# indygreg/python-zstandard

Measured on NVIDIA H100. Metric: uncompressed GB/s (compress+decompress), higher is better.
Workload: dtype u8

## Files before the change

### python_zstandard_b200/csrc/zb_common.cuh

```cuda
#pragma once
#include <cstdint>
#include <cstring>
#include <cuda_runtime.h>

typedef uint8_t  u8;
typedef uint16_t u16;
typedef uint32_t u32;
typedef uint64_t u64;

enum : u32 {
    ZB_OK = 0,
    ZB_E_GENERIC = 1,
    ZB_E_PREFIX_UNKNOWN = 10,
    ZB_E_FRAMEPARAM_UNSUPPORTED = 14,
    ZB_E_WINDOW_TOO_LARGE = 16,
    ZB_E_CORRUPTION = 20,
    ZB_E_CHECKSUM_WRONG = 22,
    ZB_E_LITERALS_HEADER_WRONG = 24,
    ZB_E_DICT_CORRUPTED = 30,
    ZB_E_DICT_WRONG = 32,
    ZB_E_TABLELOG_TOO_LARGE = 44,
    ZB_E_MAXSYMBOL_TOO_SMALL = 48,
    ZB_E_MEMORY = 64,
    ZB_E_DSTSIZE_TOO_SMALL = 70,
// ... 139 lines not shown
};

typedef uint4 ZbSeq;

typedef u32 ZbFseCell;
#define ZB_CELL(next, nb, add, sym) ((u32)(next) | ((u32)(nb) << 10) | ((u32)(add) << 14) | ((u32)(sym) << 19))
#define ZB_CELL_NEXT(c) ((c) & 1023u)
#define ZB_CELL_NB(c)   (((c) >> 10) & 15u)
#define ZB_CELL_ADD(c)  (((c) >> 14) & 31u)
#define ZB_CELL_SYM(c)  ((c) >> 19)
#define ZB_CELL16(sym, x) ((u16)((sym) | ((x) << 6)))

struct ZbDictDev {
    const u8* content; u32 content_size; u32 dict_id;
    const u16* huf; u32 huf_log; u32 has_entropy;
    const ZbFseCell* ll; const ZbFseCell* of; const ZbFseCell* ml;
    u32 ll_log, of_log, ml_log;
    u32 rep[3];
};

struct ZbDictDigest {
    u16 huf[4096]; ZbFseCell ll[512]; ZbFseCell ml[512]; ZbFseCell of[256];
    u32 huf_log, ll_log, of_log, ml_log; u32 rep[3]; u32 dict_id; u32 content_off; u32 status; u32 has_entropy; u32 pad;
    short c_norm_ll[36], c_norm_of[32], c_norm_ml[54]; u32 c_max_ll, c_max_of, c_max_ml;
    u8 c_huf_nb[256]; u32 c_huf_max;
};

__device__ __forceinline__ u32 zb_rd16(const u8* p) { return (u32)p[0] | ((u32)p[1] << 8); }
__device__ __forceinline__ u32 zb_rd24(const u8* p) { return zb_rd16(p) | ((u32)p[2] << 16); }
__device__ __forceinline__ u32 zb_rd32(const u8* p) { return zb_rd16(p) | (zb_rd16(p + 2) << 16); }
__device__ __forceinline__ u64 zb_rd64(const u8* p) { return (u64)zb_rd32(p) | ((u64)zb_rd32(p + 4) << 32); }
__device__ __forceinline__ int zb_hibit(u32 v) { return 31 - __clz(v); }

__device__ __forceinline__ void zb_cp16(u8* sdst, const u8* gsrc)
{
#ifdef __CUDA_ARCH__
    asm volatile("cp.async.cg.shared.global [%0], [%1], 16;" :: "r"((u32)__cvta_generic_to_shared(sdst)), "l"(gsrc) : "memory");
#else
    memcpy(sdst, gsrc, 16);
#endif
}
__device__ __forceinline__ void zb_cp_commit()
{
#ifdef __CUDA_ARCH__
    asm volatile("cp.async.commit_group;" ::: "memory");
#endif
}
template <int N> __device__ __forceinline__ void zb_cp_wait()
{
#ifdef __CUDA_ARCH__
    asm volatile("cp.async.wait_group %0;" :: "n"(N) : "memory");
#endif
}

#ifdef __CUDA_ARCH__
#define ZB_RING_ARG(name) u8* name
#else
#define ZB_RING_ARG(name) u8* name = nullptr
#endif
template <int D>
struct ZbBitR {
    static_assert(D >= 2 && (D & (D - 1)) == 0, "ring depth: a power of two");
    const u8* c; u8* ring; int widx; u32 hi, lo; int avail; u32 nx0, nx1; int skew_bits; int lo_c; u32 n_;
#ifndef __CUDA_ARCH__
    alignas(16) u8 own[16 * D];
#endif

    __device__ __forceinline__ u32 word(int j) const { return *(const u32*)(ring + ((u32)j & (4u * D - 1)) * 4u); }
    __device__ __forceinline__ void fetch(int k) { zb_cp16(ring + ((u32)k & (D - 1)) * 16u, c + 16 * k); }
    __device__ __forceinline__ ~ZbBitR() { zb_cp_wait<0>(); }

    __device__ __forceinline__ bool start(const u8* s, u32 n, u8* ring_) {
        if (n == 0) return false;
#ifdef __CUDA_ARCH__
        ring = ring_;
#else
        ring = ring_ ? ring_ : own;
#endif
        c = (const u8*)((uintptr_t)s & ~(uintptr_t)15);
        int const skew = (int)(s - c);
        skew_bits = skew * 8; n_ = n;
        int const top = (skew + (int)n - 1) >> 4;
        #pragma unroll
        for (int q = 0; q < D; q++) if (top - q >= 0) fetch(top - q);
        zb_cp_commit();
        lo_c = top - D + 1 > 0 ? top - D + 1 : 0;
        return true;
    }
    __device__ __forceinline__ bool finish() {
        zb_cp_wait<0>();
        int const e = skew_bits / 8 + (int)n_ - 1;
        u32 const last = ring[(u32)e & (16u * D - 1)];
        if (last == 0) return false;
        int const P = e * 8 + zb_hibit(last);
        nx0 = nx1 = 0; lo = 0;
        if (P == 0) { hi = 0; avail = 0; widx = -1; return true; }
        int const wi = (P - 1) >> 5, k = P - wi * 32;
        hi = word(wi) << (32 - k); avail = k; widx = wi - 1;
        if (widx >= 0) nx0 = word(widx);
        if (widx >= 1) nx1 = word(widx - 1);
        refill();
        return true;
    }
    __device__ __forceinline__ bool init(const u8* s, u32 n, u8* ring_) { return start(s, n, ring_) && finish(); }
    __device__ __forceinline__ void refill() {
        zb_cp_wait<4 * D - 8>();
        bool const r = (avail <= 32) & (widx >= 0);
        u32 const a = (u32)avail;
        u32 const add_hi = __funnelshift_rc(nx0, 0u, a);
        u32 const new_lo = __funnelshift_lc(0u, nx0, 32u - a);
        hi |= r ? add_hi : 0u;
        lo = r ? new_lo : lo;
        avail += r ? 32 : 0;
        widx -= r ? 1 : 0;
        nx0 = r ? nx1 : nx0;
        if (r && widx >= 1) nx1 = word(widx - 1);
        int const t = ((widx - 1) >> 2) + 1 - D;
        if (t >= 0 && t < lo_c) { fetch(t); lo_c = t; }
        zb_cp_commit();
    }
    __device__ __forceinline__ u32 peek(u32 nb) const { return __funnelshift_rc(hi, 0u, 32u - nb); }
    __device__ __forceinline__ void skip(u32 nb) {
        hi = __funnelshift_lc(lo, hi, nb); lo = __funnelshift_lc(0u, lo, nb); avail -= (int)nb;
    }
    __device__ __forceinline__ u32 read(u32 nb) { u32 const v = peek(nb); skip(nb); return v; }
    __device__ __forceinline__ int left() const { return avail + 32 * (widx + 1) - skew_bits; }
};
```

### python_zstandard_b200/csrc/zb_entropy.cuh

```cuda
#pragma once

#define ZB_ENT_WS_BYTES   256
#define ZB_ENT_WS_STRIDE  (ZB_ENT_WS_BYTES + 16)
#define ZB_ENT_SKEW(b)    ((((b) + 15u) & ~15u) | 16u)
#define ZB_ENT_DEF_LL     512
#define ZB_ENT_DEF_OF     (ZB_ENT_DEF_LL + 2 * 64)
#define ZB_ENT_DEF_ML     (ZB_ENT_DEF_OF + 2 * 32)
#define ZB_ENT_HEAD_BYTES (ZB_ENT_DEF_ML + 2 * 64)
#define ZB_ENT_POOL_BYTES(W) ((((227 * 1024 - ZB_ENT_HEAD_BYTES) / (W))) & ~15)
#define ZB_ENT_SMEM(W)    ((W) * ZB_ENT_POOL_BYTES(W) + ZB_ENT_HEAD_BYTES)

enum : u32 { ZB_SRC_NONE = 0, ZB_SRC_PREDEF = 1, ZB_SRC_RLE = 2, ZB_SRC_NCOUNT = 3, ZB_SRC_DICT = 4 };
struct ZbTabSrc { u32 kind; u32 sym; const u8* p; u32 n; };

enum : u32 { ZB_BD_FIRST = 1, ZB_BD_FSE_VALID = 2, ZB_BD_SKIP = 4 };
struct ZbBlkDesc {
    u64 hdr_off;
    u64 seq_off, lit_off;
    u32 span;
    u32 frame;
    u32 flags;
    u32 block_max;
    ZbTabSrc dHuf, dLL, dOF, dML;
};
// ... 62 lines not shown
            u32 const sy = wt[u], x = (u32)(u16)norm[sy]; norm[sy] = (short)(x + 1);
            u32 const nb = log - (u32)zb_hibit(x);
            wt[u] = (u16)(sy | (nb << 4) | (((x << nb) - size) << 8));
        }
        clear_nibbles();
        ZbBitR<4> b;
        if (!b.init(s + 1 + used, hdr - used, ring)) return 0;
        u32 s1 = b.read(log), s2 = b.read(log); b.refill();
        if (b.left() < 0) return 0;
        nsym = 0;
        for (;;) {
            if (nsym + 2 > 255) return 0;
            { u32 c = wt[s1], w = c & 15; if (w > 12) return 0; put(nsym, w); rank.count(w); total += (1u << w) >> 1; nsym++;
              s1 = (c >> 8) + b.read((c >> 4) & 15); b.refill(); }
            if (b.left() < 0) { u32 w = wt[s2] & 15; if (w > 12) return 0; put(nsym, w); rank.count(w); total += (1u << w) >> 1; nsym++; break; }
            if (nsym + 2 > 255) return 0;
            { u32 c = wt[s2], w = c & 15; if (w > 12) return 0; put(nsym, w); rank.count(w); total += (1u << w) >> 1; nsym++;
              s2 = (c >> 8) + b.read((c >> 4) & 15); b.refill(); }
            if (b.left() < 0) { u32 w = wt[s1] & 15; if (w > 12) return 0; put(nsym, w); rank.count(w); total += (1u << w) >> 1; nsym++; break; }
        }
    }
    if (total == 0) return 0;
    u32 const log = (u32)zb_hibit(total) + 1;
    if (log > 12) return 0;
    u32 const rest = (1u << log) - total, hb = (u32)zb_hibit(rest);
    if ((1u << hb) != rest) return 0;
    put(nsym, hb + 1); rank.count(hb + 1); nsym++;
    if (rank[1] < 2 || (rank[1] & 1)) return 0;
    out_log = log; out_nsym = nsym;
    return hdr + 1;
}

#define ZB_HUF_COARSE 8u
struct ZbHufTab { const u16* cells; u32 log, shift, T, base; };
__device__ __forceinline__ void zb_huf_shape(u32 log, ZbRank const& rank, u32& shift, u32& T, u32& base, u32& bytes)
{
    shift = log > ZB_HUF_COARSE ? log - ZB_HUF_COARSE : 0u;
    T = 0;
    #pragma unroll
    for (u32 wt = 1; wt <= 12 - ZB_HUF_COARSE; wt++) T += wt <= shift ? rank[wt] << (wt - 1) : 0u;
    base = (T + 3u) & ~3u;
    bytes = 2u * (base + (1u << (log - shift)));
}
__device__ __forceinline__ ZbHufTab zb_huf_full(const u16* cells, u32 log) { ZbHufTab t; t.cells = cells; t.log = log; t.shift = 0; t.T = 0; t.base = 0; return t; }
#define ZB_HCELL(t, v) ((t).cells[(v) < (t).T ? (v) : (t).base + ((v) >> (t).shift)])

__device__ static void zb_huf_fill(u16* cells, const u8* ws, u32 log, u32 nsym, ZbRank const& rank, u32 shift, u32 base)
{
    ZbPacked<6, 16> next; next.clear();
    {
        u32 p = 0;
        #pragma unroll
        for (u32 wt = 1; wt <= 12; wt++) { next.add(wt - 1, p); p += wt <= log ? (rank[wt] << (wt - 1)) : 0; }
    }
    for (u32 i = 0; i < nsym; i++) {
        u32 const wt = (ws[i >> 1] >> ((i & 1) * 4)) & 15; if (!wt) continue;
        u32 len = 1u << (wt - 1), p = next.get(wt - 1); next.add(wt - 1, len);
        if (wt > shift) { len >>= shift; p = base + (p >> shift); }
        u32 const cell = i | ((log + 1 - wt) << 8);
        if (len >= 4) { u64 const v = cell * 0x0001000100010001ull; u64* q = (u64*)(cells + p); for (u32 k = 0; k < len / 4; k++) q[k] = v; }
        else if (len == 2) *(u32*)(cells + p) = cell * 0x00010001u;
        else cells[p] = (u16)cell;
    }
}

#ifdef ZB_SIMT_EMULATION
__device__ __forceinline__ ZbRank zb_rank_pack(const u32* rank) { ZbRank r; r.clear(); for (u32 wt = 1; wt <= 12; wt++) r.add(wt - 1, rank[wt]); return r; }
__device__ static u32 zb_huf_weights(u8* ws, const u8* s, u32 n, u32& out_log, u32& out_nsym, u32* rank, ZB_RING_ARG(ring))
{
    ZbRank r; u32 const used = zb_huf_weights(ws, s, n, out_log, out_nsym, r, ring);
    rank[0] = used ? out_nsym : 0;
    for (u32 w = 1; w <= 12; w++) { rank[w] = used ? r[w] : 0; rank[0] -= rank[w]; }
    return used;
}
__device__ __forceinline__ void zb_huf_shape(u32 log, const u32* rank, u32& shift, u32& T, u32& base, u32& bytes)
{
    zb_huf_shape(log, zb_rank_pack(rank), shift, T, base, bytes);
}
__device__ static void zb_huf_fill(u16* cells, const u8* ws, u32 log, u32 nsym, const u32* rank, u32 shift, u32 base)
{
    zb_huf_fill(cells, ws, log, nsym, zb_rank_pack(rank), shift, base);
}
#endif

__device__ static bool zb_huf_stream2(u8* out, u32 n_out, const u8* s, u32 n, ZbHufTab const t, u8* ring)
{
    ZbBitR<4> b;
    if (!b.init(s, n, ring)) return false;
    u32 const log = t.log;
    u32 i = 0;
    while (i < n_out && ((uintptr_t)(out + i) & 3)) { u32 v = b.peek(log); u32 c = ZB_HCELL(t, v); out[i++] = (u8)c; b.skip(c >> 8); b.refill(); }
    for (; i + 4 <= n_out; i += 4) {
        u32 v0 = b.peek(log); u32 c0 = ZB_HCELL(t, v0); b.skip(c0 >> 8);
        u32 v1 = b.peek(log); u32 c1 = ZB_HCELL(t, v1); b.skip(c1 >> 8); b.refill();
        u32 v2 = b.peek(log); u32 c2 = ZB_HCELL(t, v2); b.skip(c2 >> 8);
        u32 v3 = b.peek(log); u32 c3 = ZB_HCELL(t, v3); b.skip(c3 >> 8); b.refill();
        *(u32*)(out + i) = (c0 & 255) | ((c1 & 255) << 8) | ((c2 & 255) << 16) | (c3 << 24);
    }
    for (; i < n_out; i++) { u32 v = b.peek(log); u32 c = ZB_HCELL(t, v); out[i] = (u8)c; b.skip(c >> 8); b.refill(); }
    return b.left() == 0;
}

struct ZbHufLane { ZbBitR<4> b; u8* out; u32 left; };

__device__ __forceinline__ void zb_huf_one(ZbHufLane& h, ZbHufTab const& t)
{
    u32 const v = h.b.peek(t.log); u32 const c = ZB_HCELL(t, v); *h.out++ = (u8)c; h.b.skip(c >> 8); h.b.refill(); h.left--;
}
#define ZB_HUF4(h) do { \
        u32 const v0_ = h.b.peek(t.log); u32 const c0_ = ZB_HCELL(t, v0_); h.b.skip(c0_ >> 8); \
        u32 const v1_ = h.b.peek(t.log); u32 const c1_ = ZB_HCELL(t, v1_); h.b.skip(c1_ >> 8); h.b.refill(); \
        u32 const v2_ = h.b.peek(t.log); u32 const c2_ = ZB_HCELL(t, v2_); h.b.skip(c2_ >> 8); \
        u32 const v3_ = h.b.peek(t.log); u32 const c3_ = ZB_HCELL(t, v3_); h.b.skip(c3_ >> 8); h.b.refill(); \
        *(u32*)h.out = (c0_ & 255) | ((c1_ & 255) << 8) | ((c2_ & 255) << 16) | (c3_ << 24); h.out += 4; h.left -= 4; } while (0)

__device__ static bool zb_huf_block(u8* dstl, u32 regen, const u8* p, u32 left, bool single, ZbHufTab const t, ZB_RING_ARG(ring))
{
    if (single) return zb_huf_stream2(dstl, regen, p, left, t, ring);
    if (left < 10) return false;
    u32 const l1 = zb_rd16(p), l2 = zb_rd16(p + 2), l3 = zb_rd16(p + 4), seg = (regen + 3) / 4;
    if (6 + l1 + l2 + l3 > left || seg * 3 > regen) return false;
    u32 const l4 = left - 6 - l1 - l2 - l3;
    ZbHufLane h0, h1, h2, h3;
    u8* const r1 = ring ? ring + 64 : nullptr; u8* const r2 = ring ? ring + 128 : nullptr; u8* const r3 = ring ? ring + 192 : nullptr;
    if (!h0.b.start(p + 6, l1, ring) || !h1.b.start(p + 6 + l1, l2, r1) || !h2.b.start(p + 6 + l1 + l2, l3, r2) || !h3.b.start(p + 6 + l1 + l2 + l3, l4, r3)) return false;
    if (!h0.b.finish() || !h1.b.finish() || !h2.b.finish() || !h3.b.finish()) return false;
    h0.out = dstl; h1.out = dstl + seg; h2.out = dstl + 2 * seg; h3.out = dstl + 3 * seg;
    h0.left = h1.left = h2.left = seg; h3.left = regen - 3 * seg;
    while (h0.left && ((uintptr_t)h0.out & 3)) zb_huf_one(h0, t);
    while (h1.left && ((uintptr_t)h1.out & 3)) zb_huf_one(h1, t);
    while (h2.left && ((uintptr_t)h2.out & 3)) zb_huf_one(h2, t);
    while (h3.left && ((uintptr_t)h3.out & 3)) zb_huf_one(h3, t);
    while (h0.left >= 4 && h1.left >= 4 && h2.left >= 4 && h3.left >= 4) { ZB_HUF4(h0); ZB_HUF4(h1); ZB_HUF4(h2); ZB_HUF4(h3); }
    while (h0.left >= 4) ZB_HUF4(h0);
    while (h1.left >= 4) ZB_HUF4(h1);
    while (h2.left >= 4) ZB_HUF4(h2);
    while (h3.left >= 4) ZB_HUF4(h3);
    while (h0.left) zb_huf_one(h0, t);
    while (h1.left) zb_huf_one(h1, t);
    while (h2.left) zb_huf_one(h2, t);
    while (h3.left) zb_huf_one(h3, t);
    return h0.b.left() == 0 && h1.b.left() == 0 && h2.b.left() == 0 && h3.b.left() == 0;
}

__device__ static int zb_seq_desc(ZbTabSrc& d, u32 mode, u32 max_sym_kind, u32 max_log, const u8* ip, u32 avail,
                                  bool repeat_ok, short* norm, u32& log, u32& max_sym, u32& need)
{
    int used = 0;
    if (mode == 0) { d.kind = ZB_SRC_PREDEF; }
    else if (mode == 1) { if (avail == 0 || ip[0] > max_sym_kind) return -1; d.kind = ZB_SRC_RLE; d.sym = ip[0]; used = 1; }
    else if (mode == 2) { d.kind = ZB_SRC_NCOUNT; d.p = ip; d.n = avail; }
    else if (!repeat_ok || d.kind == ZB_SRC_NONE) return -1;
    need = 0; log = 0; max_sym = max_sym_kind;
    if (d.kind == ZB_SRC_NCOUNT) {
        u32 const u = zb_read_ncount(norm, max_sym, log, d.p, d.n);
        if (u == 0 || log > max_log) return -1;
        if (mode == 2) { used = (int)u; d.n = u; }
        need = 2u << log;
    } else if (d.kind == ZB_SRC_RLE) need = 2;
    return used;
}

template <class F> __device__ __forceinline__ void zb_cta_for(u32 n, F f)
{
#ifdef __CUDA_ARCH__
    for (u32 i = threadIdx.x; i < n; i += blockDim.x) f(i);
#else
    if (threadIdx.x == 0) for (u32 i = 0; i < n; i++) f(i);
#endif
}

__device__ __forceinline__ void zb_cta_cells16(u8* dst, const ZbFseCell* src, u32 log)
{
    zb_cta_for(1u << log, [&](u32 i) { u32 const c = src[i]; ((u16*)dst)[i] = ZB_CELL16(ZB_CELL_SYM(c), (ZB_CELL_NEXT(c) + (1u << log)) >> ZB_CELL_NB(c)); });
}

template <int W>
__device__ __forceinline__ u32 zb_ent_head(u8* smem, ZbDictDev const& dict)
{
    u32* const lutLL = (u32*)smem; u32* const lutML = lutLL + 36;
    zb_cta_for(36, [&](u32 i) { lutLL[i] = c_LL_base[i] | ((u32)c_LL_bits[i] << 24); });
    zb_cta_for(53, [&](u32 i) { lutML[i] = c_ML_base[i] | ((u32)c_ML_bits[i] << 24); });
    zb_cta_cells16(smem + ZB_ENT_DEF_LL, g_defLL, 6);
    zb_cta_cells16(smem + ZB_ENT_DEF_OF, g_defOF, 5);
    zb_cta_cells16(smem + ZB_ENT_DEF_ML, g_defML, 6);
    u32 head = ZB_ENT_HEAD_BYTES;
    if (dict.has_entropy) {
        zb_cta_cells16(smem + head, dict.ll, dict.ll_log); head += 2u << dict.ll_log;
        zb_cta_cells16(smem + head, dict.of, dict.of_log); head += 2u << dict.of_log;
        zb_cta_cells16(smem + head, dict.ml, dict.ml_log); head += 2u << dict.ml_log;
    }
    __syncthreads();
    return ((ZB_ENT_SMEM(W) - head) / W) & ~15u;
}

#ifdef ZB_PHASE_TIMERS
__device__ unsigned long long g_zb_ent_phase[8];
#define ZB_EMARK(k) do { if (lane == 0) { long long const t_ = clock64(); atomicAdd(&g_zb_ent_phase[k], (unsigned long long)(t_ - t_ph)); t_ph = t_; } } while (0)
#elif defined(ZB_DEBUG_BLOCKS)
#define ZB_EMARK(k) do { if (err && !(t_ph & 1)) { printf("[emark %d] lane %u err %u\n", k, lane, err); t_ph |= 1; } } while (0)
#else
#define ZB_EMARK(k) do { (void)t_ph; } while (0)
#endif

template <bool SYMREP>
__device__ __forceinline__ u32 zb_seq_block(const u8* smem, u8* q, u8* ws, ZbDictDev const& dict,
                                            ZbTabSrc const& dLL, ZbTabSrc const& dOF, ZbTabSrc const& dML,
                                            u32 msLL, u32 msOF, u32 msML, u32 logLL, u32 logOF, u32 logML,
                                            const u8* ip, const u8* bend, u32 nseq, ZbSeq* sq, u32 n_lit, u64 room, u64 hist,
                                            u32& rep0, u32& rep1, u32& rep2, u32& lit_used, u32& produced, long long& t_ph)
{
    const u32* const lutLL = (const u32*)smem; const u32* const lutML = lutLL + 36;
    short* const normLL = (short*)ws; short* const normOF = normLL + 36; short* const normML = normOF + 32;
    u32 const dct_ll = ZB_ENT_HEAD_BYTES, dct_of = dct_ll + (2u << dict.ll_log), dct_ml = dct_of + (2u << dict.of_log);
    ZbTab tLL, tOF, tML;
    auto setup = [&](const ZbTabSrc& d, short* norm, u32 ms, u32 lg, int kind, u32 dct, u32 dlog, u32 def, u32 deflog, ZbTab& t) {
        if (d.kind == ZB_SRC_NCOUNT) { zb_build_fse((u16*)q, norm, ms, lg, kind); t.off = (u32)(q - smem); t.log = lg; q += 2u << lg; }
        else if (d.kind == ZB_SRC_RLE) { *(u16*)q = ZB_CELL16(d.sym, 1u); t.off = (u32)(q - smem); t.log = 0; q += 2; }
        else if (d.kind == ZB_SRC_DICT) { t.off = dct; t.log = dlog; }
        else { t.off = def; t.log = deflog; }
    };
    setup(dLL, normLL, msLL, logLL, K_LL, dct_ll, dict.ll_log, ZB_ENT_DEF_LL, 6, tLL);
    setup(dOF, normOF, msOF, logOF, K_OF, dct_of, dict.of_log, ZB_ENT_DEF_OF, 5, tOF);
// ... 40 lines not shown
        if (slow) b.refill();
        {
            u32 const both = b.read(ab);
            ml += both >> llb; ll += both & ((1u << llb) - 1);
        }
        if (slow) b.refill();
        {
            u32 const v = b.read(sb);
            sLL = (xl << nl) - (1u << tLL.log) + (v >> (nm + no));
            sML = (xm << nm) - (1u << tML.log) + ((v >> no) & ((1u << nm) - 1));
            sOF = (xo << no) - (1u << tOF.log) + (v & ((1u << no) - 1));
        }
        sq[i] = make_uint4(lit_used, produced, ml, off);
        if ((u64)produced + ll + ml > room) { err = ZB_E_DSTSIZE_TOO_SMALL; break; }
        if (ll > n_lit - lit_used) { err = ZB_E_CORRUPTION; break; }
        lit_used += ll; produced += ll;
        if ((u64)off > hist + produced) { err = ZB_E_CORRUPTION; break; }
        produced += ml;
    }
    if (!err && b.left() != 0) err = ZB_E_CORRUPTION;
    return err;
}

template <int ZB_ENT_WARPS>
__global__ void __launch_bounds__(ZB_ENT_WARPS * 32)
zb_entropy_decode(const u8* __restrict__ src, const ZbSegment* __restrict__ segs, u32 n_frames,
                  const ZbFramePlace* __restrict__ place, const u64* __restrict__ dst_sizes,
                  ZbBlock* __restrict__ blocks, ZbSeq* __restrict__ seqs, u8* __restrict__ lits,
                  u32* __restrict__ work_counter, ZbDictDev dict, u32* status, u64* __restrict__ out_sizes,
                  u32* __restrict__ ck_expect, u32 take)
{
    ZB_DYN_SMEM(zb_smem);
    u32 const lane = threadIdx.x & 31, warp = threadIdx.x >> 5;
    u32 const pool_bytes = zb_ent_head<ZB_ENT_WARPS>(zb_smem, dict);
    u8* const pool = zb_smem + ZB_ENT_SMEM(ZB_ENT_WARPS) - (ZB_ENT_WARPS - warp) * pool_bytes;
    u8* const ws = pool + lane * ZB_ENT_WS_STRIDE;
    u8* const tabs = pool + 32 * ZB_ENT_WS_STRIDE;
    u32 const TAB_BYTES = pool_bytes - 32 * ZB_ENT_WS_STRIDE;

    for (;;) {
        u32 base = 0;
        if (lane == 0) base = atomicAdd(work_counter, take);
        base = __shfl_sync(0xFFFFFFFFu, base, 0);
        if (base >= n_frames) return;
        u32 const f = base + lane;
        bool done = lane >= take || !(f < n_frames) || status[f] != ZB_OK;

        const u8* s = src; u64 n = 0; ZbHdr h; ZbFramePlace pl; u32 err = ZB_OK;
        u64 cap = 0, out_pos = 0, blk_i = 0, seq_i = 0, lit_i = 0, pos = 0; u32 block_max = 0;
        u32 rep0 = 1, rep1 = 4, rep2 = 8;
        ZbTabSrc dHuf = {ZB_SRC_NONE, 0, nullptr, 0}, dLL = dHuf, dOF = dHuf, dML = dHuf;
        bool fse_valid = false;
        if (!done) {
            s = src + segs[f].offset; n = segs[f].length;
            zb_skip_skippable(s, n);
            zb_parse_header(s, n, h);
            pl = place[f]; cap = pl.dst_cap; blk_i = pl.blk_off; seq_i = pl.seq_off; lit_i = pl.lit_off; pos = h.hdr_size;
            block_max = h.window < ZB_BLOCK_MAX ? (u32)h.window : ZB_BLOCK_MAX;
            if (dict.has_entropy) {
                dHuf.kind = dLL.kind = dOF.kind = dML.kind = ZB_SRC_DICT; fse_valid = true;
                rep0 = dict.rep[0]; rep1 = dict.rep[1]; rep2 = dict.rep[2];
            }
            if (h.dict_id && dict.dict_id && h.dict_id != dict.dict_id) { err = ZB_E_DICT_WRONG; done = true; }
        }
        u64 const hist_extra = dict.content_size;

        long long t_ph = clock64() & ~1ll;
// ... 28 lines not shown
                        B.n_lit = L.regen; comp = true;
                    }
                } while (0);
                if (err) { done = true; comp = false; }
            }
            ZB_EMARK(1);
            bool wantH = false; u32 hlog = 0, hns = 0; ZbRank rank; const u8* hp = nullptr; u32 hleft = 0;
            if (comp) {
                do {
                    if (L.type == 0) {
                        if (L.hdr + L.regen > bsize) { err = ZB_E_CORRUPTION; break; }
                        B.lit_kind = ZB_LIT_RAW; B.src_pos = (u64)(bs + L.hdr - src); ip = bs + L.hdr + L.regen;
                    } else if (L.type == 1) {
                        if (L.hdr + 1 > bsize) { err = ZB_E_CORRUPTION; break; }
                        B.lit_kind = ZB_LIT_RLE; B.lit_byte = bs[L.hdr]; ip = bs + L.hdr + 1;
                    } else {
                        if (L.type == 3 && dHuf.kind == ZB_SRC_NONE) { err = ZB_E_DICT_CORRUPTED; break; }
                        if (!L.single && L.regen < 6) { err = ZB_E_LITERALS_HEADER_WRONG; break; }
                        if (L.csize + L.hdr > bsize || L.regen == 0) { err = ZB_E_CORRUPTION; break; }
                        hp = bs + L.hdr; hleft = L.csize;
                        if (L.type == 2) { dHuf.kind = ZB_SRC_NCOUNT; dHuf.p = hp; dHuf.n = hleft; }
                        if (dHuf.kind == ZB_SRC_NCOUNT) {
                            u32 const used = zb_huf_weights(ws, dHuf.p, dHuf.n, hlog, hns, rank, tabs + lane * 80);
                            if (used == 0 || (L.type == 2 && used >= hleft)) { err = ZB_E_CORRUPTION; break; }
                            if (L.type == 2) { hp += used; hleft -= used; dHuf.n = used; }
                            wantH = true;
                        }
                        B.lit_kind = ZB_LIT_SCRATCH; B.src_pos = lit_i; ip = bs + L.hdr + L.csize;
                    }
                } while (0);
                if (err) { done = true; comp = false; wantH = false; }
            }
            if (comp && B.lit_kind == ZB_LIT_SCRATCH && dHuf.kind == ZB_SRC_DICT) {
                if (!zb_huf_block(lits + lit_i, L.regen, hp, hleft, L.single, zb_huf_full(dict.huf, dict.huf_log), ws)) { err = ZB_E_CORRUPTION; done = true; comp = false; }
            }
            ZB_EMARK(2);
            {
                bool pending = wantH;
                u32 hshift = 0, hT = 0, hbase = 0, hbytes = 0;
                if (wantH) zb_huf_shape(hlog, rank, hshift, hT, hbase, hbytes);
                while (__any_sync(0xFFFFFFFFu, pending)) {
                    u32 const need = pending ? hbytes : 0;
                    u32 const incl = zb_warp_incl_scan((need + 15) & ~15u, lane);
                    if (pending && incl <= TAB_BYTES) {
                        u16* cells = (u16*)(tabs + incl - ((need + 15) & ~15u));
                        zb_huf_fill(cells, ws, hlog, hns, rank, hshift, hbase);
                        ZB_EMARK(6);
                        ZbHufTab t; t.cells = cells; t.log = hlog; t.shift = hshift; t.T = hT; t.base = hbase;
                        if (!zb_huf_block(lits + lit_i, L.regen, hp, hleft, L.single, t, ws)) { err = ZB_E_CORRUPTION; done = true; comp = false; }
                        pending = false;
                    }
                    __syncwarp();
                }
            }
            ZB_EMARK(3);
            if (comp && B.lit_kind == ZB_LIT_SCRATCH) lit_i += (L.regen + 15) & ~15u;
            u32 nseq = 0, logLL = 0, logOF = 0, logML = 0, msLL = 0, msOF = 0, msML = 0, needS = 0;
            short* const normLL = (short*)ws; short* const normOF = normLL + 36; short* const normML = normOF + 32;
            if (comp) {
                do {
                    if (ip >= bend) { err = ZB_E_SRCSIZE_WRONG; break; }
                    nseq = *ip++;
                    if (nseq > 0x7F) {
                        if (nseq == 0xFF) { if (ip + 2 > bend) { err = ZB_E_SRCSIZE_WRONG; break; } nseq = zb_rd16(ip) + 0x7F00; ip += 2; }
                        else { if (ip >= bend) { err = ZB_E_SRCSIZE_WRONG; break; } nseq = ((nseq - 0x80) << 8) + *ip++; }
                    }
                    B.n_seq = nseq;
                    if (nseq == 0) { if (ip != bend) err = ZB_E_CORRUPTION; break; }
                    if (ip + 1 > bend) { err = ZB_E_SRCSIZE_WRONG; break; }
                    u32 const modes = *ip++;
                    if (modes & 3) { err = ZB_E_CORRUPTION; break; }
                    u32 nd; int r;
                    r = zb_seq_desc(dLL, modes >> 6, 35, 9, ip, (u32)(bend - ip), fse_valid, normLL, logLL, msLL, nd);
                    if (r < 0) { err = ZB_E_CORRUPTION; break; } ip += r; needS += nd;
                    r = zb_seq_desc(dOF, (modes >> 4) & 3, 31, 8, ip, (u32)(bend - ip), fse_valid, normOF, logOF, msOF, nd);
                    if (r < 0) { err = ZB_E_CORRUPTION; break; } ip += r; needS += nd;
                    r = zb_seq_desc(dML, (modes >> 2) & 3, 52, 9, ip, (u32)(bend - ip), fse_valid, normML, logML, msML, nd);
                    if (r < 0) { err = ZB_E_CORRUPTION; break; } ip += r; needS += nd;
                    fse_valid = true;
                } while (0);
                if (err) { done = true; comp = false; nseq = 0; }
// ... 26 lines not shown
                    if (!err && B.regen > block_max) err = ZB_E_CORRUPTION;
                    pos += bsize;
                }
                if (!err) {
                    blocks[blk_i++] = B;
                    out_pos += B.regen;
                    if (last) {
                        if (h.content_size != ZB_CONTENT_UNKNOWN && out_pos != h.content_size) err = ZB_E_CORRUPTION;
                        else if (h.checksum && pos + 4 > n) err = ZB_E_CHECKSUM_WRONG;
                        else {
                            if (h.checksum) ck_expect[f] = zb_rd32(s + pos);
                            if (dst_sizes && out_pos != cap) err = ZB_E_SIZE_MISMATCH;
                        }
                        done = true;
                    }
                }
                if (err) done = true;
            }
        }
        if (lane < take && f < n_frames && status[f] == ZB_OK) {
            if (err) { status[f] = err; out_sizes[f] = err == ZB_E_SIZE_MISMATCH ? out_pos : 0; } else out_sizes[f] = out_pos;
        } else if (lane < take && f < n_frames) out_sizes[f] = 0;
    }
}

template <int ZB_ENT_WARPS>
__global__ void __launch_bounds__(ZB_ENT_WARPS * 32)
zb_entropy_blocks(const u8* __restrict__ src, const ZbBlkDesc* __restrict__ bdesc, u32 n_blocks,
                  ZbBlock* __restrict__ blocks, ZbSeq* __restrict__ seqs, u8* __restrict__ lits,
                  u32* __restrict__ work_counter, ZbDictDev dict, u32* status, ZbBlkExit* __restrict__ bexit, u32 take)
{
    ZB_DYN_SMEM(zb_smem);
    u32 const lane = threadIdx.x & 31, warp = threadIdx.x >> 5;
    u32 const pool_bytes = zb_ent_head<ZB_ENT_WARPS>(zb_smem, dict);
    u8* const pool = zb_smem + ZB_ENT_SMEM(ZB_ENT_WARPS) - (ZB_ENT_WARPS - warp) * pool_bytes;
    u8* const ws = pool + lane * ZB_ENT_WS_BYTES;
    u8* const tabs = pool + 32 * ZB_ENT_WS_BYTES;
    u32 const TAB_BYTES = pool_bytes - 32 * ZB_ENT_WS_BYTES;

    for (;;) {
        u32 base = 0;
        if (lane == 0) base = atomicAdd(work_counter, take);
        base = __shfl_sync(0xFFFFFFFFu, base, 0);
        if (base >= n_blocks) return;
        u32 const bi = base + lane;
        ZbBlkDesc D; D.frame = 0; D.flags = 0;
        if (lane < take && bi < n_blocks) D = bdesc[bi];
        bool done = lane >= take || !(bi < n_blocks) || (D.flags & ZB_BD_SKIP) || status[D.frame] != ZB_OK;

        const u8* s = src; u64 n = 0; u32 err = ZB_OK;
        u64 const cap = ~0ull >> 1; u64 out_pos = 0, blk_i = bi, seq_i = 0, lit_i = 0, pos = 0; u32 block_max = 0;
        u32 rep0 = 1, rep1 = 4, rep2 = 8;
        ZbTabSrc dHuf = {ZB_SRC_NONE, 0, nullptr, 0}, dLL = dHuf, dOF = dHuf, dML = dHuf;
        bool fse_valid = false;
        if (!done) {
            s = src + D.hdr_off; n = D.span; seq_i = D.seq_off; lit_i = D.lit_off; block_max = D.block_max;
            dHuf = D.dHuf; dLL = D.dLL; dOF = D.dOF; dML = D.dML; fse_valid = (D.flags & ZB_BD_FSE_VALID) != 0;
            if (D.flags & ZB_BD_FIRST) { if (dict.has_entropy) { rep0 = dict.rep[0]; rep1 = dict.rep[1]; rep2 = dict.rep[2]; } }
            else { rep0 = 0x80000000u; rep1 = 0xA0000000u; rep2 = 0xC0000000u; }
        }
        u64 const hist_extra = 1ull << 40;

        long long t_ph = clock64() & ~1ll;
        while (__any_sync(0xFFFFFFFFu, !done)) {
            ZB_EMARK(0);
            ZbBlock B; B.kind = 0; B.regen = 0; B.n_seq = 0; B.n_lit = 0; B.lit_kind = 0; B.lit_byte = 0; B.src_pos = 0; B.seq_pos = seq_i; B.out_pos = out_pos;
            bool comp = false, last = false;
// ... 24 lines not shown
                        B.n_lit = L.regen; comp = true;
                    }
                } while (0);
                if (err) { done = true; comp = false; }
            }
            ZB_EMARK(1);
            bool wantH = false; u32 hlog = 0, hns = 0; ZbRank rank; const u8* hp = nullptr; u32 hleft = 0;
            if (comp) {
                do {
                    if (L.type == 0) {
                        if (L.hdr + L.regen > bsize) { err = ZB_E_CORRUPTION; break; }
                        B.lit_kind = ZB_LIT_RAW; B.src_pos = (u64)(bs + L.hdr - src); ip = bs + L.hdr + L.regen;
                    } else if (L.type == 1) {
                        if (L.hdr + 1 > bsize) { err = ZB_E_CORRUPTION; break; }
                        B.lit_kind = ZB_LIT_RLE; B.lit_byte = bs[L.hdr]; ip = bs + L.hdr + 1;
                    } else {
                        if (L.type == 3 && dHuf.kind == ZB_SRC_NONE) { err = ZB_E_DICT_CORRUPTED; break; }
                        if (!L.single && L.regen < 6) { err = ZB_E_LITERALS_HEADER_WRONG; break; }
                        if (L.csize + L.hdr > bsize || L.regen == 0) { err = ZB_E_CORRUPTION; break; }
                        hp = bs + L.hdr; hleft = L.csize;
                        if (L.type == 2) { dHuf.kind = ZB_SRC_NCOUNT; dHuf.p = hp; dHuf.n = hleft; }
                        if (dHuf.kind == ZB_SRC_NCOUNT) {
                            u32 const used = zb_huf_weights(ws, dHuf.p, dHuf.n, hlog, hns, rank, tabs + lane * 64);
                            if (used == 0 || (L.type == 2 && used >= hleft)) { err = ZB_E_CORRUPTION; break; }
                            if (L.type == 2) { hp += used; hleft -= used; dHuf.n = used; }
                            wantH = true;
                        }
                        B.lit_kind = ZB_LIT_SCRATCH; B.src_pos = lit_i; ip = bs + L.hdr + L.csize;
                    }
                } while (0);
                if (err) { done = true; comp = false; wantH = false; }
            }
            if (comp && B.lit_kind == ZB_LIT_SCRATCH && dHuf.kind == ZB_SRC_DICT) {
                if (!zb_huf_block(lits + lit_i, L.regen, hp, hleft, L.single, zb_huf_full(dict.huf, dict.huf_log), ws)) { err = ZB_E_CORRUPTION; done = true; comp = false; }
            }
            ZB_EMARK(2);
            {
                bool pending = wantH;
                u32 hshift = 0, hT = 0, hbase = 0, hbytes = 0;
                if (wantH) zb_huf_shape(hlog, rank, hshift, hT, hbase, hbytes);
                while (__any_sync(0xFFFFFFFFu, pending)) {
                    u32 const need = pending ? hbytes : 0;
                    u32 const incl = zb_warp_incl_scan((need + 15) & ~15u, lane);
                    if (pending && incl <= TAB_BYTES) {
                        u16* cells = (u16*)(tabs + incl - ((need + 15) & ~15u));
                        zb_huf_fill(cells, ws, hlog, hns, rank, hshift, hbase);
                        ZB_EMARK(6);
                        ZbHufTab t; t.cells = cells; t.log = hlog; t.shift = hshift; t.T = hT; t.base = hbase;
                        if (!zb_huf_block(lits + lit_i, L.regen, hp, hleft, L.single, t, ws)) { err = ZB_E_CORRUPTION; done = true; comp = false; }
                        pending = false;
                    }
                    __syncwarp();
                }
            }
            ZB_EMARK(3);
            if (comp && B.lit_kind == ZB_LIT_SCRATCH) lit_i += (L.regen + 15) & ~15u;
            u32 nseq = 0, logLL = 0, logOF = 0, logML = 0, msLL = 0, msOF = 0, msML = 0, needS = 0;
            short* const normLL = (short*)ws; short* const normOF = normLL + 36; short* const normML = normOF + 32;
            if (comp) {
                do {
                    if (ip >= bend) { err = ZB_E_SRCSIZE_WRONG; break; }
                    nseq = *ip++;
                    if (nseq > 0x7F) {
                        if (nseq == 0xFF) { if (ip + 2 > bend) { err = ZB_E_SRCSIZE_WRONG; break; } nseq = zb_rd16(ip) + 0x7F00; ip += 2; }
                        else { if (ip >= bend) { err = ZB_E_SRCSIZE_WRONG; break; } nseq = ((nseq - 0x80) << 8) + *ip++; }
                    }
                    B.n_seq = nseq;
                    if (nseq == 0) { if (ip != bend) err = ZB_E_CORRUPTION; break; }
                    if (ip + 1 > bend) { err = ZB_E_SRCSIZE_WRONG; break; }
                    u32 const modes = *ip++;
                    if (modes & 3) { err = ZB_E_CORRUPTION; break; }
                    u32 nd; int r;
                    r = zb_seq_desc(dLL, modes >> 6, 35, 9, ip, (u32)(bend - ip), fse_valid, normLL, logLL, msLL, nd);
                    if (r < 0) { err = ZB_E_CORRUPTION; break; } ip += r; needS += nd;
                    r = zb_seq_desc(dOF, (modes >> 4) & 3, 31, 8, ip, (u32)(bend - ip), fse_valid, normOF, logOF, msOF, nd);
                    if (r < 0) { err = ZB_E_CORRUPTION; break; } ip += r; needS += nd;
                    r = zb_seq_desc(dML, (modes >> 2) & 3, 52, 9, ip, (u32)(bend - ip), fse_valid, normML, logML, msML, nd);
                    if (r < 0) { err = ZB_E_CORRUPTION; break; } ip += r; needS += nd;
                    fse_valid = true;
                } while (0);
                if (err) { done = true; comp = false; nseq = 0; }
// ... 46 lines not shown
```

Before: 147.0.

## Rework Huffman literal decoder with batched reload bit reader and shared-memory tables

```diff
diff --git a/python_zstandard_b200/csrc/zb_common.cuh b/python_zstandard_b200/csrc/zb_common.cuh
--- a/python_zstandard_b200/csrc/zb_common.cuh
+++ b/python_zstandard_b200/csrc/zb_common.cuh
@@ -195,6 +195,53 @@
 __device__ __forceinline__ u64 zb_rd64(const u8* p) { return (u64)zb_rd32(p) | ((u64)zb_rd32(p + 4) << 32); }
 __device__ __forceinline__ int zb_hibit(u32 v) { return 31 - __clz(v); }
 
+#ifdef __CUDA_ARCH__
+typedef u32 ZbSmem;
+__device__ __forceinline__ ZbSmem zb_smem_addr(const void* p) { return (u32)__cvta_generic_to_shared(p); }
+__device__ __forceinline__ u32 zb_lds16(ZbSmem a) { u16 v; asm("ld.shared.u16 %0, [%1];" : "=h"(v) : "r"(a)); return v; }
+__device__ __forceinline__ u32 zb_lds32(ZbSmem a) { u32 v; asm volatile("ld.shared.u32 %0, [%1];" : "=r"(v) : "r"(a)); return v; }
+#else
+struct ZbSmem {
+    u8* p;
+    ZbSmem() = default;
+    ZbSmem(const void* q) : p((u8*)q) {}
+    ZbSmem operator+(u32 o) const { return ZbSmem(p + o); }
+};
+__device__ __forceinline__ ZbSmem zb_smem_addr(const void* p) { return ZbSmem(p); }
+__device__ __forceinline__ u32 zb_lds16(ZbSmem a) { return *(const u16*)a.p; }
+__device__ __forceinline__ u32 zb_lds32(ZbSmem a) { return *(const u32*)a.p; }
+#endif
+
+#if !defined(__CUDA_ARCH__) && defined(ZB_SIMT_EMULATION)
+#include <deque>
+#include <vector>
+struct ZbCpCopy { u8* dst; const u8* src; };
+struct ZbCpThread { std::deque<std::vector<ZbCpCopy>> groups; std::vector<ZbCpCopy> open; };
+static std::vector<ZbCpThread> zb_cp_threads;
+static unsigned long long zb_cp_early_reads = 0;
+static inline ZbCpThread& zb_cp_self()
+{
+    size_t const t = (size_t)simt::g_cur;
+    if (zb_cp_threads.size() <= t) zb_cp_threads.resize(t + 1);
+    return zb_cp_threads[t];
+}
+static inline void zb_cp16(u8* sdst, const u8* gsrc) { zb_cp_self().open.push_back(ZbCpCopy{sdst, gsrc}); memset(sdst, 0xA5, 16); }
+static inline void zb_cp_commit() { ZbCpThread& T = zb_cp_self(); T.groups.push_back(std::move(T.open)); T.open.clear(); }
+template <int N> static inline void zb_cp_wait()
+{
+    ZbCpThread& T = zb_cp_self();
+    while (T.groups.size() > (size_t)N) { for (ZbCpCopy const& c : T.groups.front()) memcpy(c.dst, c.src, 16); T.groups.pop_front(); }
+}
+static inline u32 zb_cp_read32(const u8* p)
+{
+    ZbCpThread& T = zb_cp_self();
+    bool early = false;
+    for (auto const& g : T.groups) for (ZbCpCopy const& c : g) early |= p + 4 > c.dst && p < c.dst + 16;
+    for (ZbCpCopy const& c : T.open) early |= p + 4 > c.dst && p < c.dst + 16;
+    zb_cp_early_reads += early;
+    return *(const u32*)p;
+}
+#else
 __device__ __forceinline__ void zb_cp16(u8* sdst, const u8* gsrc)
 {
 #ifdef __CUDA_ARCH__
@@ -215,6 +262,18 @@
     asm volatile("cp.async.wait_group %0;" :: "n"(N) : "memory");
 #endif
 }
+__device__ __forceinline__ u32 zb_cp_read32(const u8* p) { return *(const u32*)p; }
+#endif
+#ifdef __CUDA_ARCH__
+__device__ __forceinline__ void zb_cp16(ZbSmem sdst, const u8* gsrc)
+{
+    asm volatile("cp.async.cg.shared.global [%0], [%1], 16;" :: "r"(sdst), "l"(gsrc) : "memory");
+}
+__device__ __forceinline__ u32 zb_ring_read32(ZbSmem a) { return zb_lds32(a); }
+#else
+__device__ __forceinline__ void zb_cp16(ZbSmem sdst, const u8* gsrc) { zb_cp16(sdst.p, gsrc); }
+__device__ __forceinline__ u32 zb_ring_read32(ZbSmem a) { return zb_cp_read32(a.p); }
+#endif
 
 #ifdef __CUDA_ARCH__
 #define ZB_RING_ARG(name) u8* name
@@ -229,7 +288,7 @@
     alignas(16) u8 own[16 * D];
 #endif
 
-    __device__ __forceinline__ u32 word(int j) const { return *(const u32*)(ring + ((u32)j & (4u * D - 1)) * 4u); }
+    __device__ __forceinline__ u32 word(int j) const { return zb_cp_read32(ring + ((u32)j & (4u * D - 1)) * 4u); }
     __device__ __forceinline__ void fetch(int k) { zb_cp16(ring + ((u32)k & (D - 1)) * 16u, c + 16 * k); }
     __device__ __forceinline__ ~ZbBitR() { zb_cp_wait<0>(); }
 
@@ -289,3 +348,60 @@
     __device__ __forceinline__ u32 read(u32 nb) { u32 const v = peek(nb); skip(nb); return v; }
     __device__ __forceinline__ int left() const { return avail + 32 * (widx + 1) - skew_bits; }
 };
+
+#define ZB_HUF_RING 4
+#define ZB_HUF_LAG  ((32 * (4 * ZB_HUF_RING - 7) - 31 + 47) / 48 - 1)
+#ifndef ZB_HUF_WAIT_SHORT
+#define ZB_HUF_WAIT_SHORT 0
+#endif
+struct ZbHufR {
+    static constexpr int D = ZB_HUF_RING;
+    const u8* c; ZbSmem ring; u32 hi, lo; int P, end, lo_c; u32 n_;
+#ifndef __CUDA_ARCH__
+    alignas(16) u8 own[16 * D];
+#endif
+
+    __device__ __forceinline__ u32 word(int j) const { return zb_ring_read32(ring + ((u32)j & (4u * D - 1)) * 4u); }
+    __device__ __forceinline__ ~ZbHufR() { zb_cp_wait<0>(); }
+
+    __device__ __forceinline__ bool start(const u8* s, u32 n, u8* ring_) {
+        if (n == 0) return false;
+#ifdef __CUDA_ARCH__
+        ring = zb_smem_addr(ring_);
+#else
+        ring = ring_ ? ring_ : own;
+#endif
+        c = (const u8*)((uintptr_t)s & ~(uintptr_t)15);
+        end = (int)(s - c) * 8; n_ = n;
+        int const top = (int)((s - c) + n - 1) >> 4;
+        #pragma unroll
+        for (int q = 0; q < D; q++) if (top - q >= 0) zb_cp16(ring + (u32)((top - q) & (D - 1)) * 16u, c + 16 * (top - q));
+        zb_cp_commit();
+        lo_c = top - D + 1 > 0 ? top - D + 1 : 0;
+        return true;
+    }
+    __device__ __forceinline__ bool finish() {
+        zb_cp_wait<0>();
+        int const e = end / 8 + (int)n_ - 1;
+        u32 const last = (word(e >> 2) >> ((e & 3) * 8)) & 255u;
+        if (last == 0) return false;
+        P = e * 8 + zb_hibit(last);
+        return true;
+    }
+    __device__ __forceinline__ bool init(const u8* s, u32 n, u8* ring_) { return start(s, n, ring_) && finish(); }
+    __device__ __forceinline__ int reload() {
+        int const w = (P - 1) >> 5;
+        u32 const sh = (u32)~(P - 1) & 31u;
+        u32 const w0 = word(w), w1 = word(w - 1), w2 = word(w - 2);
+        hi = __funnelshift_lc(w1, w0, sh); lo = __funnelshift_lc(w2, w1, sh);
+        return w;
+    }
+    __device__ __forceinline__ void fetch(int w) {
+        int const t = (w >> 2) + 1 - D;
+        if (t >= 0 && t < lo_c) { zb_cp16(ring + (u32)(t & (D - 1)) * 16u, c + 16 * t); lo_c = t; }
+    }
+    __device__ __forceinline__ u32 peek(u32 sh) const { return hi >> sh; }
+    __device__ __forceinline__ void skip(u32 nb) { hi = __funnelshift_lc(lo, hi, nb); lo <<= nb; P -= (int)nb; }
+    __device__ __forceinline__ int left() const { return P - end; }
+};
+template <int N> __device__ __forceinline__ void zb_huf_wait() { zb_cp_wait<N + ZB_HUF_WAIT_SHORT>(); }
diff --git a/python_zstandard_b200/csrc/zb_entropy.cuh b/python_zstandard_b200/csrc/zb_entropy.cuh
--- a/python_zstandard_b200/csrc/zb_entropy.cuh
+++ b/python_zstandard_b200/csrc/zb_entropy.cuh
@@ -118,7 +118,7 @@
 }
 
 #define ZB_HUF_COARSE 8u
-struct ZbHufTab { const u16* cells; u32 log, shift, T, base; };
+struct ZbHufTab { ZbSmem cells; u32 log, shift, T, base; };
 __device__ __forceinline__ void zb_huf_shape(u32 log, ZbRank const& rank, u32& shift, u32& T, u32& base, u32& bytes)
 {
     shift = log > ZB_HUF_COARSE ? log - ZB_HUF_COARSE : 0u;
@@ -128,8 +128,7 @@
     base = (T + 3u) & ~3u;
     bytes = 2u * (base + (1u << (log - shift)));
 }
-__device__ __forceinline__ ZbHufTab zb_huf_full(const u16* cells, u32 log) { ZbHufTab t; t.cells = cells; t.log = log; t.shift = 0; t.T = 0; t.base = 0; return t; }
-#define ZB_HCELL(t, v) ((t).cells[(v) < (t).T ? (v) : (t).base + ((v) >> (t).shift)])
+#define ZB_HCELL(t, v) zb_lds16((t).cells + 2u * ((v) < (t).T ? (v) : (t).base + ((v) >> (t).shift)))
 
 __device__ static void zb_huf_fill(u16* cells, const u8* ws, u32 log, u32 nsym, ZbRank const& rank, u32 shift, u32 base)
 {
@@ -169,36 +168,42 @@
 }
 #endif
 
+struct ZbHufLane { ZbHufR b; u8* out; u32 left; };
+
+__device__ __forceinline__ u32 zb_huf_sym(ZbHufR& b, ZbHufTab const& t, u32 sh)
+{
+    u32 const v = b.peek(sh); u32 const c = ZB_HCELL(t, v); b.skip(c >> 8); return c & 255u;
+}
+__device__ __forceinline__ void zb_huf_put4(ZbHufLane& h, u32 c0, u32 c1, u32 c2, u32 c3)
+{
+    *(u32*)h.out = c0 | (c1 << 8) | (c2 << 16) | (c3 << 24); h.out += 4; h.left -= 4;
+}
+__device__ __forceinline__ void zb_huf_one(ZbHufLane& h, ZbHufTab const& t, u32 sh)
+{
+    zb_huf_wait<ZB_HUF_LAG>(); int const w = h.b.reload(); *h.out++ = (u8)zb_huf_sym(h.b, t, sh); h.left--; h.b.fetch(w); zb_cp_commit();
+}
+__device__ __forceinline__ void zb_huf_tail(ZbHufLane& h, ZbHufTab const& t, u32 sh)
+{
+    while (h.left >= 4) {
+        zb_huf_wait<ZB_HUF_LAG>();
+        int const w = h.b.reload();
+        u32 const c0 = zb_huf_sym(h.b, t, sh), c1 = zb_huf_sym(h.b, t, sh), c2 = zb_huf_sym(h.b, t, sh), c3 = zb_huf_sym(h.b, t, sh);
+        zb_huf_put4(h, c0, c1, c2, c3);
+        h.b.fetch(w); zb_cp_commit();
+    }
+    while (h.left) zb_huf_one(h, t, sh);
+}
+
 __device__ static bool zb_huf_stream2(u8* out, u32 n_out, const u8* s, u32 n, ZbHufTab const t, u8* ring)
 {
-    ZbBitR<4> b;
-    if (!b.init(s, n, ring)) return false;
-    u32 const log = t.log;
-    u32 i = 0;
-    while (i < n_out && ((uintptr_t)(out + i) & 3)) { u32 v = b.peek(log); u32 c = ZB_HCELL(t, v); out[i++] = (u8)c; b.skip(c >> 8); b.refill(); }
-    for (; i + 4 <= n_out; i += 4) {
-        u32 v0 = b.peek(log); u32 c0 = ZB_HCELL(t, v0); b.skip(c0 >> 8);
-        u32 v1 = b.peek(log); u32 c1 = ZB_HCELL(t, v1); b.skip(c1 >> 8); b.refill();
-        u32 v2 = b.peek(log); u32 c2 = ZB_HCELL(t, v2); b.skip(c2 >> 8);
-        u32 v3 = b.peek(log); u32 c3 = ZB_HCELL(t, v3); b.skip(c3 >> 8); b.refill();
-        *(u32*)(out + i) = (c0 & 255) | ((c1 & 255) << 8) | ((c2 & 255) << 16) | (c3 << 24);
-    }
-    for (; i < n_out; i++) { u32 v = b.peek(log); u32 c = ZB_HCELL(t, v); out[i] = (u8)c; b.skip(c >> 8); b.refill(); }
-    return b.left() == 0;
-}
-
-struct ZbHufLane { ZbBitR<4> b; u8* out; u32 left; };
-
-__device__ __forceinline__ void zb_huf_one(ZbHufLane& h, ZbHufTab const& t)
-{
-    u32 const v = h.b.peek(t.log); u32 const c = ZB_HCELL(t, v); *h.out++ = (u8)c; h.b.skip(c >> 8); h.b.refill(); h.left--;
-}
-#define ZB_HUF4(h) do { \
-        u32 const v0_ = h.b.peek(t.log); u32 const c0_ = ZB_HCELL(t, v0_); h.b.skip(c0_ >> 8); \
-        u32 const v1_ = h.b.peek(t.log); u32 const c1_ = ZB_HCELL(t, v1_); h.b.skip(c1_ >> 8); h.b.refill(); \
-        u32 const v2_ = h.b.peek(t.log); u32 const c2_ = ZB_HCELL(t, v2_); h.b.skip(c2_ >> 8); \
-        u32 const v3_ = h.b.peek(t.log); u32 const c3_ = ZB_HCELL(t, v3_); h.b.skip(c3_ >> 8); h.b.refill(); \
-        *(u32*)h.out = (c0_ & 255) | ((c1_ & 255) << 8) | ((c2_ & 255) << 16) | (c3_ << 24); h.out += 4; h.left -= 4; } while (0)
+    ZbHufLane h;
+    if (!h.b.init(s, n, ring)) return false;
+    u32 const sh = 32 - t.log;
+    h.out = out; h.left = n_out;
+    while (h.left && ((uintptr_t)h.out & 3)) zb_huf_one(h, t, sh);
+    zb_huf_tail(h, t, sh);
+    return h.b.left() == 0;
+}
 
 __device__ static bool zb_huf_block(u8* dstl, u32 regen, const u8* p, u32 left, bool single, ZbHufTab const t, ZB_RING_ARG(ring))
 {
@@ -211,21 +216,25 @@
     u8* const r1 = ring ? ring + 64 : nullptr; u8* const r2 = ring ? ring + 128 : nullptr; u8* const r3 = ring ? ring + 192 : nullptr;
     if (!h0.b.start(p + 6, l1, ring) || !h1.b.start(p + 6 + l1, l2, r1) || !h2.b.start(p + 6 + l1 + l2, l3, r2) || !h3.b.start(p + 6 + l1 + l2 + l3, l4, r3)) return false;
     if (!h0.b.finish() || !h1.b.finish() || !h2.b.finish() || !h3.b.finish()) return false;
+    u32 const sh = 32 - t.log;
     h0.out = dstl; h1.out = dstl + seg; h2.out = dstl + 2 * seg; h3.out = dstl + 3 * seg;
     h0.left = h1.left = h2.left = seg; h3.left = regen - 3 * seg;
-    while (h0.left && ((uintptr_t)h0.out & 3)) zb_huf_one(h0, t);
-    while (h1.left && ((uintptr_t)h1.out & 3)) zb_huf_one(h1, t);
-    while (h2.left && ((uintptr_t)h2.out & 3)) zb_huf_one(h2, t);
-    while (h3.left && ((uintptr_t)h3.out & 3)) zb_huf_one(h3, t);
-    while (h0.left >= 4 && h1.left >= 4 && h2.left >= 4 && h3.left >= 4) { ZB_HUF4(h0); ZB_HUF4(h1); ZB_HUF4(h2); ZB_HUF4(h3); }
-    while (h0.left >= 4) ZB_HUF4(h0);
-    while (h1.left >= 4) ZB_HUF4(h1);
-    while (h2.left >= 4) ZB_HUF4(h2);
-    while (h3.left >= 4) ZB_HUF4(h3);
-    while (h0.left) zb_huf_one(h0, t);
-    while (h1.left) zb_huf_one(h1, t);
-    while (h2.left) zb_huf_one(h2, t);
-    while (h3.left) zb_huf_one(h3, t);
+    while (h0.left && ((uintptr_t)h0.out & 3)) zb_huf_one(h0, t, sh);
+    while (h1.left && ((uintptr_t)h1.out & 3)) zb_huf_one(h1, t, sh);
+    while (h2.left && ((uintptr_t)h2.out & 3)) zb_huf_one(h2, t, sh);
+    while (h3.left && ((uintptr_t)h3.out & 3)) zb_huf_one(h3, t, sh);
+    while (h0.left >= 4 && h1.left >= 4 && h2.left >= 4 && h3.left >= 4) {
+        zb_huf_wait<ZB_HUF_LAG>();
+        int const w0 = h0.b.reload(), w1 = h1.b.reload(), w2 = h2.b.reload(), w3 = h3.b.reload();
+        u32 const a0 = zb_huf_sym(h0.b, t, sh), a1 = zb_huf_sym(h1.b, t, sh), a2 = zb_huf_sym(h2.b, t, sh), a3 = zb_huf_sym(h3.b, t, sh);
+        u32 const b0 = zb_huf_sym(h0.b, t, sh), b1 = zb_huf_sym(h1.b, t, sh), b2 = zb_huf_sym(h2.b, t, sh), b3 = zb_huf_sym(h3.b, t, sh);
+        u32 const c0 = zb_huf_sym(h0.b, t, sh), c1 = zb_huf_sym(h1.b, t, sh), c2 = zb_huf_sym(h2.b, t, sh), c3 = zb_huf_sym(h3.b, t, sh);
+        u32 const d0 = zb_huf_sym(h0.b, t, sh), d1 = zb_huf_sym(h1.b, t, sh), d2 = zb_huf_sym(h2.b, t, sh), d3 = zb_huf_sym(h3.b, t, sh);
+        zb_huf_put4(h0, a0, b0, c0, d0); zb_huf_put4(h1, a1, b1, c1, d1); zb_huf_put4(h2, a2, b2, c2, d2); zb_huf_put4(h3, a3, b3, c3, d3);
+        h0.b.fetch(w0); h1.b.fetch(w1); h2.b.fetch(w2); h3.b.fetch(w3);
+        zb_cp_commit();
+    }
+    zb_huf_tail(h0, t, sh); zb_huf_tail(h1, t, sh); zb_huf_tail(h2, t, sh); zb_huf_tail(h3, t, sh);
     return h0.b.left() == 0 && h1.b.left() == 0 && h2.b.left() == 0 && h3.b.left() == 0;
 }
 
@@ -262,8 +271,9 @@
 }
 
 template <int W>
-__device__ __forceinline__ u32 zb_ent_head(u8* smem, ZbDictDev const& dict)
-{
+__device__ __forceinline__ u32 zb_ent_head(u8* smem, ZbDictDev const& dict, ZbHufTab& dhuf)
+{
+    dhuf.cells = zb_smem_addr(smem); dhuf.log = dhuf.shift = dhuf.T = dhuf.base = 0;
     u32* const lutLL = (u32*)smem; u32* const lutML = lutLL + 36;
     zb_cta_for(36, [&](u32 i) { lutLL[i] = c_LL_base[i] | ((u32)c_LL_bits[i] << 24); });
     zb_cta_for(53, [&](u32 i) { lutML[i] = c_ML_base[i] | ((u32)c_ML_bits[i] << 24); });
@@ -275,6 +285,15 @@
         zb_cta_cells16(smem + head, dict.ll, dict.ll_log); head += 2u << dict.ll_log;
         zb_cta_cells16(smem + head, dict.of, dict.of_log); head += 2u << dict.of_log;
         zb_cta_cells16(smem + head, dict.ml, dict.ml_log); head += 2u << dict.ml_log;
+        u32 const log = dict.huf_log, shift = log > ZB_HUF_COARSE ? log - ZB_HUF_COARSE : 0u;
+        u32 T = 0;
+        if (shift) { u32 hi = 1u << log; while (T < hi) { u32 const m = (T + hi) >> 1; if ((dict.huf[m] >> 8) > ZB_HUF_COARSE) T = m + 1; else hi = m; } }
+        u32 const base = (T + 3u) & ~3u;
+        u16* const cells = (u16*)(smem + head);
+        zb_cta_for(T, [&](u32 i) { cells[i] = dict.huf[i]; });
+        zb_cta_for(1u << (log - shift), [&](u32 j) { cells[base + j] = dict.huf[j << shift]; });
+        dhuf.cells = zb_smem_addr(cells); dhuf.log = log; dhuf.shift = shift; dhuf.T = T; dhuf.base = base;
+        head += (2u * (base + (1u << (log - shift))) + 15u) & ~15u;
     }
     __syncthreads();
     return ((ZB_ENT_SMEM(W) - head) / W) & ~15u;
@@ -381,7 +400,8 @@
 {
     ZB_DYN_SMEM(zb_smem);
     u32 const lane = threadIdx.x & 31, warp = threadIdx.x >> 5;
-    u32 const pool_bytes = zb_ent_head<ZB_ENT_WARPS>(zb_smem, dict);
+    ZbHufTab dhuf;
+    u32 const pool_bytes = zb_ent_head<ZB_ENT_WARPS>(zb_smem, dict, dhuf);
     u8* const pool = zb_smem + ZB_ENT_SMEM(ZB_ENT_WARPS) - (ZB_ENT_WARPS - warp) * pool_bytes;
     u8* const ws = pool + lane * ZB_ENT_WS_STRIDE;
     u8* const tabs = pool + 32 * ZB_ENT_WS_STRIDE;
@@ -476,7 +496,7 @@
                 if (err) { done = true; comp = false; wantH = false; }
             }
             if (comp && B.lit_kind == ZB_LIT_SCRATCH && dHuf.kind == ZB_SRC_DICT) {
-                if (!zb_huf_block(lits + lit_i, L.regen, hp, hleft, L.single, zb_huf_full(dict.huf, dict.huf_log), ws)) { err = ZB_E_CORRUPTION; done = true; comp = false; }
+                if (!zb_huf_block(lits + lit_i, L.regen, hp, hleft, L.single, dhuf, ws)) { err = ZB_E_CORRUPTION; done = true; comp = false; }
             }
             ZB_EMARK(2);
             {
@@ -490,7 +510,7 @@
                         u16* cells = (u16*)(tabs + incl - ((need + 15) & ~15u));
                         zb_huf_fill(cells, ws, hlog, hns, rank, hshift, hbase);
                         ZB_EMARK(6);
-                        ZbHufTab t; t.cells = cells; t.log = hlog; t.shift = hshift; t.T = hT; t.base = hbase;
+                        ZbHufTab t; t.cells = zb_smem_addr(cells); t.log = hlog; t.shift = hshift; t.T = hT; t.base = hbase;
                         if (!zb_huf_block(lits + lit_i, L.regen, hp, hleft, L.single, t, ws)) { err = ZB_E_CORRUPTION; done = true; comp = false; }
                         pending = false;
                     }
@@ -583,7 +603,8 @@
 {
     ZB_DYN_SMEM(zb_smem);
     u32 const lane = threadIdx.x & 31, warp = threadIdx.x >> 5;
-    u32 const pool_bytes = zb_ent_head<ZB_ENT_WARPS>(zb_smem, dict);
+    ZbHufTab dhuf;
+    u32 const pool_bytes = zb_ent_head<ZB_ENT_WARPS>(zb_smem, dict, dhuf);
     u8* const pool = zb_smem + ZB_ENT_SMEM(ZB_ENT_WARPS) - (ZB_ENT_WARPS - warp) * pool_bytes;
     u8* const ws = pool + lane * ZB_ENT_WS_BYTES;
     u8* const tabs = pool + 32 * ZB_ENT_WS_BYTES;
@@ -674,7 +695,7 @@
                 if (err) { done = true; comp = false; wantH = false; }
             }
             if (comp && B.lit_kind == ZB_LIT_SCRATCH && dHuf.kind == ZB_SRC_DICT) {
-                if (!zb_huf_block(lits + lit_i, L.regen, hp, hleft, L.single, zb_huf_full(dict.huf, dict.huf_log), ws)) { err = ZB_E_CORRUPTION; done = true; comp = false; }
+                if (!zb_huf_block(lits + lit_i, L.regen, hp, hleft, L.single, dhuf, ws)) { err = ZB_E_CORRUPTION; done = true; comp = false; }
             }
             ZB_EMARK(2);
             {
@@ -688,7 +709,7 @@
                         u16* cells = (u16*)(tabs + incl - ((need + 15) & ~15u));
                         zb_huf_fill(cells, ws, hlog, hns, rank, hshift, hbase);
                         ZB_EMARK(6);
-                        ZbHufTab t; t.cells = cells; t.log = hlog; t.shift = hshift; t.T = hT; t.base = hbase;
+                        ZbHufTab t; t.cells = zb_smem_addr(cells); t.log = hlog; t.shift = hshift; t.T = hT; t.base = hbase;
                         if (!zb_huf_block(lits + lit_i, L.regen, hp, hleft, L.single, t, ws)) { err = ZB_E_CORRUPTION; done = true; comp = false; }
                         pending = false;
                     }
```

Result: no change. 146.2, median of 6 (-0.5%).
